# NJU-LHRS/LHRS-Bot

Measured on AMD Instinct MI355X. Metric: stage-1 pretrain samples/sec (224^2 image + 128-tok caption), higher is better.
Workload: dtype bf16

## Files before the change

### include/lhrs_hip.h

```cpp
#ifndef LHRS_HIP_H
#define LHRS_HIP_H
#include <stdint.h>
#ifdef __cplusplus
extern "C" {
#endif

typedef uint16_t lhrs_bf16_t;

const char* lhrs_last_error(void);
int lhrs_abi_version(void);
const char* lhrs_target_arch(void);

int lhrs_gemm_bf16_nt(const void* A, int lda, const void* B, int ldb, void* C, int ldc, int M, int N, int K,
                      const void* bias, const void* residual, int ldr, int act, int out_f32, int accumulate,
                      float alpha, void* stream);

int lhrs_gemm_bf16_nt_lora(const void* A, int lda, const void* B, int ldb, const void* A2, int lda2, const void* B2, int ldb2,
                           int K2, void* C, int ldc, int M, int N, int K, const void* bias, const void* residual, int ldr,
                           int out_f32, int accumulate, float alpha, void* stream);
int lhrs_gemm_fp8_nt(const void* A8, long lda, const float* sa, const void* B8, long ldb, const float* sb, void* C, int ldc,
                     int M, int N, int K, const void* residual, int ldr, float alpha, void* stream);
int lhrs_gemm_fp8_nt_lora(const void* A8, long lda, const float* sa, const void* B8, long ldb, const float* sb, const void* A2,
                          int lda2, const void* B2, int ldb2, int K2, void* C, int ldc, int M, int N, int K,
                          const void* residual, int ldr, float alpha, void* stream);
// ... 72 lines not shown
int lhrs_layernorm_fwd(const void* x, long ldx, const void* gamma, const void* beta, void* y, long ldy, float* mean,
                       float* rstd, int rows, int cols, float eps, void* stream);
int lhrs_layernorm_bwd_nblk(int rows);
int lhrs_layernorm_bwd(const void* dy, long ld_dy, const void* x, long ldx, const void* gamma, const float* mean,
                       const float* rstd, const void* add, void* dx, long ld_dx, float* dgamma, float* dbeta,
                       float* partial, int accumulate, int rows, int cols, void* stream);
int lhrs_rmsnorm_fwd(const void* x, long ldx, const void* w, void* y, long ldy, float* rstd, int rows, int cols,
                     float eps, void* stream);
int lhrs_rmsnorm_bwd(const void* dy, const void* x, const void* w, const float* rstd, const void* add, void* dx,
                     int rows, int cols, float eps, void* stream);

int lhrs_seq_transpose(const void* in, long ld_in, void* out, int cols, int LT, const int* desc, int nseq, int use_kv,
                       void* stream);
int lhrs_attn_fwd(const void* q, long ldq, const void* k, long ldk, const void* v, long ldv, void* o, long ldo, float* lse,
                  const int* desc, int nseq, int H, int D, int max_q, int max_kv, int LTq, int causal, float scale,
                  void* stream);
int lhrs_attn_fwd_kmask(const void* q, long ldq, const void* k, long ldk, const void* v, long ldv, void* o, long ldo,
                        float* lse, const int* desc, int nseq, int H, int D, int max_q, int max_kv, int LTq,
                        int causal, float scale, const unsigned char* key_mask, long ld_mask, void* stream);
int lhrs_attn_delta(const void* o, long ldo, const void* dout, long ld_do, float* delta, const int* desc, int nseq, int H,
                    int D, int max_q, int LTq, void* stream);
int lhrs_attn_bwd(const void* q, long ldq, const void* k, long ldk, const void* v, long ldv, const void* dout,
                  long ld_do, const float* lse, const float* delta, void* dq, long ld_dq, void* dk, long ld_dk, void* dv,
                  long ld_dv, const int* desc, int nseq, int H, int D, int max_q, int max_kv, int LTq, int causal,
                  float scale, void* stream);
int lhrs_attn_bwd_rope(const void* q, long ldq, const void* k, long ldk, const void* v, long ldv, const void* dout,
                       long ld_do, const float* lse, const float* delta, void* dq, long ld_dq, void* dk, long ld_dk, void* dv,
                       long ld_dv, const int* desc, int nseq, int H, int D, int max_q, int max_kv, int LTq, int causal,
                       float scale, const float* cos_t, const float* sin_t, int pos_mod, int pos0, long rows, void* stream);
int lhrs_attn_bwd_o(const void* q, long ldq, const void* k, long ldk, const void* v, long ldv, const void* dout, long ld_do,
                    const void* o, long ldo, const float* lse, float* delta, void* dq, long ld_dq, void* dk, long ld_dk, void* dv,
                    long ld_dv, const int* desc, int nseq, int H, int D, int max_q, int max_kv, int LTq, int causal, float scale,
                    const float* cos_t, const float* sin_t, int pos_mod, int pos0, long rows, void* stream);

int lhrs_patchify(const float* rgb, void* out, int B, int img, int P, int KP, void* stream);
int lhrs_vit_assemble(const void* patch, const void* cls, const void* pos, void* out, int B, int NP, int dim,
                      void* stream);
int lhrs_rope(void* x, long ld, int rows, int nheads, int D, const float* cos_t, const float* sin_t, const int* pos_ids,
              int pos_mod, int pos0, int inverse, void* stream);
int lhrs_swiglu_fwd(const void* gate_up, void* act, long rows, int F, void* stream);
int lhrs_swiglu_bwd(const void* dact, const void* gate_up, void* dgate_up, long rows, int F, void* stream);
int lhrs_map(int op, const void* a, const void* b, void* out, long n, void* stream);
int lhrs_colsum_nsplit(int rows);
int lhrs_colsum(const void* x, long ld, float* out, float* partial, int rows, int cols, int accumulate, void* stream);
int lhrs_cast_f32_to_bf16(const float* in, void* out, long n, void* stream);
int lhrs_cast_bf16_to_f32(const void* in, float* out, long n, void* stream);
int lhrs_transpose(const void* in, long ld_in, void* out, long ld_out, int rows, int cols, int rows_pad, void* stream);
int lhrs_transpose_batched(const long* desc, int n, int total_tiles, void* stream);

int lhrs_pooler_build(const void* query, const void* img, void* t, void* kv, int B, int nq0, int nq1, int nq2, int ni0,
                      int ni1, int ni2, int dim, void* stream);
int lhrs_pooler_query_grad(const void* dt0, const void* dkv, float* dquery, int B, int nq0, int nq1, int nq2, int ni0,
                           int ni1, int ni2, int dim, int accumulate, void* stream);
int lhrs_copy_2d(void* dst, long dst_pitch_bytes, const void* src, long src_pitch_bytes, long width_bytes, long height,
                 void* stream);
int lhrs_debug_poison_lds(unsigned pattern, void* stream);

int lhrs_splice_fwd(const long* ids, const long* labels, const uint8_t* mask, const void* image, const void* embed,
                    void* out_embeds, long* out_labels, uint8_t* out_mask, int* img_pos, int B, int T, int NI, int dim,
                    int S, int vocab, void* stream);
int lhrs_splice_bwd(const void* d_embeds, const int* img_pos, void* d_image, int B, int NI, int dim, int S, void* stream);
int lhrs_splice_map_fwd(const long* ids, const int* src_tok, const int* src_img, const void* image, const void* embed, void* out_embeds, int B,
                        int T, int dim, int S, int vocab, void* stream);
int lhrs_splice_map_bwd(const void* d_embeds, const int* inv, void* d_image, int n_rows, int dim, void* stream);
int lhrs_gather_rows(const void* src, long ld_src, const int* idx, void* dst, long ld_dst, int n, int dim, void* stream);
int lhrs_scatter_rows(const void* src, long ld_src, const int* idx, void* dst, long ld_dst, int n, int dim, void* stream);
// ... 72 lines not shown
```

### lhrs_bot_amd/csrc/attention.hip

```cpp
#include "common.h"
#include <type_traits>

namespace {

struct AttnArgs {
  const bf16_t* q; const bf16_t* k; const bf16_t* v; const bf16_t* dout;
  long ldq, ldk, ldv, ldo, ld_do, ld_dq, ld_dk, ld_dv;
  bf16_t* o; bf16_t* dq; bf16_t* dk; bf16_t* dv;
  int LTq;
  float* lse;
  const float* delta;
  const int* desc;
  int H;
  float scale;
  const unsigned char* kmask;
  long ld_kmask;
  const float* rope_cos;
  const float* rope_sin;
  int rope_mod, rope_pos0;
  const bf16_t* o_in;
  long ld_oin;
  float* delta_w;
  int wide;
};

constexpr float NEG_INF = -__builtin_huge_valf();

template <int D>
__device__ __forceinline__ int swz(int row) {
  return D == 128 ? (((row & 7) << 1) | ((row >> 3) & 1)) : (row & 7);
}
template <int D>
__device__ __forceinline__ int rm_off(int row, int c) { return row * (D * 2) + ((c ^ swz<D>(row)) << 4); }

template <int D> struct TileRegs { uint4 v[64 * (D / 8) / 256]; };

template <int D>
__device__ __forceinline__ void tile_load(TileRegs<D>& r, const bf16_t* base, long ld, int row0, int len, int tid) {
  constexpr int CH = D / 8, N = 64 * CH / 256;
#pragma unroll
  for (int i = 0; i < N; ++i) {
    const int idx = tid + i * 256;
    const int gr = min(row0 + idx / CH, len - 1);
    r.v[i] = *reinterpret_cast<const uint4*>(base + (long)gr * ld + (idx % CH) * 8);
  }
}
template <int D>
__device__ __forceinline__ void tile_store(char* lds, const TileRegs<D>& r, int tid) {
  constexpr int CH = D / 8, N = 64 * CH / 256;
#pragma unroll
  for (int i = 0; i < N; ++i) {
    const int idx = tid + i * 256;
    *reinterpret_cast<uint4*>(lds + rm_off<D>(idx / CH, idx % CH)) = r.v[i];
  }
}
template <int D>
// ... 388 lines not shown
    for (int db = 0; db < DB; ++db) dv[db] = MFMA(join(alo[db], ahi[db]), p1, dv[db]);
    tr_wait<DB>(blo, bhi);
#pragma unroll
    for (int db = 0; db < DB; ++db) dk[db] = MFMA(join(blo[db], bhi[db]), d1, dk[db]);
  }
  if (key < kv_rows) {
    bf16_t* pk = a.dk + (long)(kv_off + key) * a.ld_dk + h * D + fg * 4;
    bf16_t* pv = a.dv + (long)(kv_off + key) * a.ld_dv + h * D + fg * 4;
#pragma unroll
    for (int db = 0; db < DB; ++db) { store4bf(pk + db * 16, dk[db], 1.f); store4bf(pv + db * 16, dv[db], 1.f); }
  }
}

template <int D> constexpr int res_rows() { return 163840 / (2 * D * 2); }

template <int D>
__device__ __forceinline__ void res_load(char* lds, const bf16_t* base, long ld, int rows, int len, int lane, int wave) {
  constexpr int CH = D / 8, R = 1024 / (D * 2);
  typedef const __attribute__((address_space(1))) void* gp;
  typedef __attribute__((address_space(3))) void* lp;
  for (int r0 = wave * R; r0 < rows; r0 += 8 * R) {
    const int row = r0 + lane / CH;
    const int c = (lane % CH) ^ swz<D>(row);
    const bf16_t* src = base + (long)min(row, len - 1) * ld + c * 8;
    __builtin_amdgcn_global_load_lds((gp)src, (lp)(lds + r0 * (D * 2)), 16, 0, 0);
  }
}
__device__ __forceinline__ int zigzag_group(int p, int wave, int G, bool descending) {
  const int k = p * 8 + ((p & 1) ? 7 - wave : wave);
  if (k >= G) return -1;
  return descending ? G - 1 - k : k;
}

#ifdef ATTN_DIAG
__device__ unsigned long long* g_attn_dbg = nullptr;
__device__ int g_attn_dbg_sel = 0;
#define DIAG_T(slot) do { if (g_attn_dbg && g_attn_dbg_sel == DIAG_KID && lane == 0) g_attn_dbg[((long)(blockIdx.y * gridDim.x + blockIdx.x) * 8 + wave) * 8 + (slot)] = wall_clock64(); } while (0)
#define DIAG_DECL(id) constexpr int DIAG_KID = id; unsigned long long dg_t = 0, dg_acc[3] = {0, 0, 0}; int dg_units = 0
#define DIAG_MARK() do { asm volatile("s_waitcnt vmcnt(0) lgkmcnt(0)" ::: "memory"); dg_t = wall_clock64(); } while (0)
#define DIAG_ACC(k) do { asm volatile("s_waitcnt vmcnt(0) lgkmcnt(0)" ::: "memory"); const unsigned long long t_ = wall_clock64(); dg_acc[k] += t_ - dg_t; dg_t = t_; } while (0)
#define DIAG_UNITS(n) dg_units += (n)
#define DIAG_FLUSH() do { if (g_attn_dbg && g_attn_dbg_sel == DIAG_KID && lane == 0) { unsigned long long* d_ = g_attn_dbg + ((long)(blockIdx.y * gridDim.x + blockIdx.x) * 8 + wave) * 8; d_[2] = dg_acc[0]; d_[3] = dg_acc[1]; d_[5] = dg_acc[2]; d_[6] = dg_units; } } while (0)
#else
#define DIAG_T(slot) do { } while (0)
#define DIAG_DECL(id)
#define DIAG_MARK() do { } while (0)
#define DIAG_ACC(k) do { } while (0)
#define DIAG_UNITS(n) do { } while (0)
#define DIAG_FLUSH() do { } while (0)
#endif

template <int D, bool CAUSAL>
__global__ __launch_bounds__(512, 2) void attn_fwd_res_kernel(AttnArgs a) {
  constexpr int KS = D / 32, DB = D / 16, TILE = 64 * D * 2;
  __shared__ __attribute__((aligned(16))) char smem[163840];
  char* lds_k = smem;
  char* lds_v = smem + res_rows<D>() * D * 2;
  const int seq = blockIdx.y, h = blockIdx.x;
  const int* ds = a.desc + seq * 8;
  const int q_off = ds[0], q_len = ds[1], kv_off = ds[2], kv_len = ds[3], coff = ds[5];
  const int tid = threadIdx.x, lane = tid & 63, fr = lane & 15, fg = lane >> 4;
  const int wave = __builtin_amdgcn_readfirstlane(tid >> 6);
  DIAG_DECL(0);
  DIAG_T(0);
  int kv_need = kv_len;
  if (CAUSAL) kv_need = max(0, min(kv_len, q_len + coff));
  const int rows = ((kv_need + 63) >> 6) << 6;
  if (rows > 0) {
    res_load<D>(lds_k, a.k + (long)kv_off * a.ldk + h * D, a.ldk, rows, kv_len, lane, wave);
    res_load<D>(lds_v, a.v + (long)kv_off * a.ldv + h * D, a.ldv, rows, kv_len, lane, wave);
  }
  asm volatile("s_waitcnt vmcnt(0)" ::: "memory");
  __syncthreads();
  DIAG_T(1);
  TrAddr<D> tv;
  tv.init(lds_v, lane);
  const float c2 = a.scale * 1.4426950408889634f;
  const int G = (q_len + 15) >> 4;
  for (int p = 0;; ++p) {
    const int g = zigzag_group(p, wave, G, CAUSAL);
    if (g < 0) break;
    DIAG_MARK();
    const int qrow = g * 16 + fr;
    const bf16_t* qp = a.q + (long)(q_off + min(qrow, q_len - 1)) * a.ldq + h * D;
    bf16x8 qf[KS];
#pragma unroll
    for (int ks = 0; ks < KS; ++ks) qf[ks] = *reinterpret_cast<const bf16x8*>(qp + ks * 32 + fg * 8);
    DIAG_ACC(0);
    float m = NEG_INF, l = 0.f;
    f32x4 o[DB];
#pragma unroll
    for (int i = 0; i < DB; ++i) o[i] = f32x4{0.f, 0.f, 0.f, 0.f};
    int kv_end = kv_len;
    if (CAUSAL) kv_end = max(0, min(kv_len, min(g * 16 + 16, q_len) + coff));
    const int ntiles = (kv_end + 63) >> 6;
    for (int j = 0; j < ntiles; ++j) {
      const char* kt = lds_k + j * TILE;
      f32x4 s[4];
#pragma unroll
      for (int nb = 0; nb < 4; ++nb) {
        s[nb] = f32x4{0.f, 0.f, 0.f, 0.f};
#pragma unroll
        for (int ks = 0; ks < KS; ++ks) s[nb] = MFMA(frag_rm<D>(kt, nb * 16 + fr, ks, fg), qf[ks], s[nb]);
      }
      TrAddr<D> tj;
#pragma unroll
      for (int db = 0; db < DB; ++db) tj.base[db] = tv.base[db] + j * TILE;
      bf16x4 v0lo[DB], v0hi[DB], v1lo[DB], v1hi[DB];
      tr_issue<D, 0>(tj, v0lo, v0hi);
      const bool full = (j + 1) * 64 <= kv_len && (!CAUSAL || j * 64 + 63 <= g * 16 + coff);
// ... 24 lines not shown
        for (int r = 0; r < 4; ++r) {
          s[nb][r] = __builtin_amdgcn_exp2f(__builtin_fmaf(s[nb][r], c2, -mc));
          rs += s[nb][r];
        }
      l = l * alpha + rs;
      m = m_new;
#pragma unroll
      for (int i = 0; i < DB; ++i) o[i] *= alpha;
      const bf16x8 p0 = pack_frag(s[0], s[1]), p1 = pack_frag(s[2], s[3]);
      tr_wait<DB>(v0lo, v0hi);
      tr_issue<D, 1>(tj, v1lo, v1hi);
      __builtin_amdgcn_sched_barrier(0);
#pragma unroll
      for (int db = 0; db < DB; ++db) o[db] = MFMA(join(v0lo[db], v0hi[db]), p0, o[db]);
      tr_wait<DB>(v1lo, v1hi);
#pragma unroll
      for (int db = 0; db < DB; ++db) o[db] = MFMA(join(v1lo[db], v1hi[db]), p1, o[db]);
    }
    DIAG_ACC(1);
    DIAG_UNITS(ntiles);
    l = group_sum(l);
    if (qrow < q_len) {
      const float inv = l > 0.f ? 1.f / l : 0.f;
      bf16_t* op = a.o + (long)(q_off + qrow) * a.ldo + h * D;
      if (a.wide) store_row_wide<DB>(op, o, inv, fg);
      else {
#pragma unroll
        for (int db = 0; db < DB; ++db) store4bf(op + fg * 4 + db * 16, o[db], inv);
      }
      if (a.lse && fg == 0) a.lse[(long)(seq * a.H + h) * a.LTq + qrow] = (l > 0.f) ? m * a.scale + __logf(l) : NEG_INF;
    }
    DIAG_ACC(2);
  }
  DIAG_T(4);
  DIAG_FLUSH();
}

template <int D, bool CAUSAL>
__global__ __launch_bounds__(512, 2) void attn_bwd_dq_res_kernel(AttnArgs a) {
  constexpr int KS = D / 32, DB = D / 16, TILE = 64 * D * 2;
  __shared__ __attribute__((aligned(16))) char smem[163840];
  char* lds_k = smem;
  char* lds_v = smem + res_rows<D>() * D * 2;
  const int seq = blockIdx.y, h = blockIdx.x;
  const int* ds = a.desc + seq * 8;
  const int q_off = ds[0], q_len = ds[1], kv_off = ds[2], kv_len = ds[3], coff = ds[5];
  const int tid = threadIdx.x, lane = tid & 63, fr = lane & 15, fg = lane >> 4;
  const int wave = __builtin_amdgcn_readfirstlane(tid >> 6);
  DIAG_DECL(1);
  DIAG_T(0);
  int kv_need = kv_len;
  if (CAUSAL) kv_need = max(0, min(kv_len, q_len + coff));
  const int rows = ((kv_need + 63) >> 6) << 6;
  if (rows > 0) {
    res_load<D>(lds_k, a.k + (long)kv_off * a.ldk + h * D, a.ldk, rows, kv_len, lane, wave);
    res_load<D>(lds_v, a.v + (long)kv_off * a.ldv + h * D, a.ldv, rows, kv_len, lane, wave);
  }
  asm volatile("s_waitcnt vmcnt(0)" ::: "memory");
  __syncthreads();
  DIAG_T(1);
  TrAddr<D> tk;
  tk.init(lds_k, lane);
  const int G = (q_len + 15) >> 4;
  for (int p = 0;; ++p) {
    const int g = zigzag_group(p, wave, G, CAUSAL);
    if (g < 0) break;
    DIAG_MARK();
    const int qrow = g * 16 + fr;
    const int qrow_c = min(qrow, q_len - 1);
    const bf16_t* qp = a.q + (long)(q_off + qrow_c) * a.ldq + h * D;
    const bf16_t* dop = a.dout + (long)(q_off + qrow_c) * a.ld_do + h * D;
    bf16x8 qf[KS], dof[KS];
#pragma unroll
    for (int ks = 0; ks < KS; ++ks) {
      qf[ks] = *reinterpret_cast<const bf16x8*>(qp + ks * 32 + fg * 8);
      dof[ks] = *reinterpret_cast<const bf16x8*>(dop + ks * 32 + fg * 8);
    }
    const long stat = (long)(seq * a.H + h) * a.LTq + qrow_c;
    float delta_q;
    if (a.o_in != nullptr) {
      const bf16_t* op = a.o_in + (long)(q_off + qrow_c) * a.ld_oin + h * D;
      float part = 0.f;
#pragma unroll
      for (int ks = 0; ks < KS; ++ks) {
        const bf16x8 of = *reinterpret_cast<const bf16x8*>(op + ks * 32 + fg * 8);
#pragma unroll
        for (int e = 0; e < 8; ++e) part += bf2f((bf16_t)dof[ks][e]) * bf2f((bf16_t)of[e]);
      }
      delta_q = group_sum(part);
      if (fg == 0 && qrow < q_len) a.delta_w[stat] = delta_q;
    } else {
      delta_q = a.delta[stat];
    }
    const float lse2 = a.lse[stat] * 1.4426950408889634f, c2 = a.scale * 1.4426950408889634f;
    DIAG_ACC(0);
    f32x4 dq[DB];
#pragma unroll
    for (int i = 0; i < DB; ++i) dq[i] = f32x4{0.f, 0.f, 0.f, 0.f};
    int kv_end = kv_len;
    if (CAUSAL) kv_end = max(0, min(kv_len, min(g * 16 + 16, q_len) + coff));
    const int ntiles = (kv_end + 63) >> 6;
    for (int j = 0; j < ntiles; ++j) {
      const char* kt = lds_k + j * TILE;
      const char* vt = lds_v + j * TILE;
      f32x4 s[4], dp[4];
#pragma unroll
      for (int nb = 0; nb < 4; ++nb) {
        s[nb] = f32x4{0.f, 0.f, 0.f, 0.f};
        dp[nb] = f32x4{0.f, 0.f, 0.f, 0.f};
#pragma unroll
        for (int ks = 0; ks < KS; ++ks) {
          s[nb] = MFMA(frag_rm<D>(kt, nb * 16 + fr, ks, fg), qf[ks], s[nb]);
          dp[nb] = MFMA(frag_rm<D>(vt, nb * 16 + fr, ks, fg), dof[ks], dp[nb]);
        }
      }
      TrAddr<D> tj;
#pragma unroll
      for (int db = 0; db < DB; ++db) tj.base[db] = tk.base[db] + j * TILE;
      bf16x4 k0lo[DB], k0hi[DB], k1lo[DB], k1hi[DB];
      tr_issue<D, 0>(tj, k0lo, k0hi);
      const bool full = (j + 1) * 64 <= kv_len && (!CAUSAL || j * 64 + 63 <= g * 16 + coff);
      if (full) {
#pragma unroll
        for (int nb = 0; nb < 4; ++nb)
#pragma unroll
          for (int r = 0; r < 4; ++r) {
            const float pv = __builtin_amdgcn_exp2f(__builtin_fmaf(s[nb][r], c2, -lse2));
// ... 5 lines not shown
#pragma unroll
          for (int r = 0; r < 4; ++r) {
            const int key = j * 64 + nb * 16 + fg * 4 + r;
            const bool ok = key < kv_len && (!CAUSAL || key <= qrow + coff) && qrow < q_len;
            const float pv = __builtin_amdgcn_exp2f(__builtin_fmaf(s[nb][r], c2, -lse2));
            s[nb][r] = ok ? pv * (dp[nb][r] - delta_q) : 0.f;
          }
      }
      const bf16x8 d0 = pack_frag(s[0], s[1]), d1 = pack_frag(s[2], s[3]);
      tr_wait<DB>(k0lo, k0hi);
      tr_issue<D, 1>(tj, k1lo, k1hi);
      __builtin_amdgcn_sched_barrier(0);
#pragma unroll
      for (int db = 0; db < DB; ++db) dq[db] = MFMA(join(k0lo[db], k0hi[db]), d0, dq[db]);
      tr_wait<DB>(k1lo, k1hi);
#pragma unroll
      for (int db = 0; db < DB; ++db) dq[db] = MFMA(join(k1lo[db], k1hi[db]), d1, dq[db]);
    }
    DIAG_ACC(1);
    DIAG_UNITS(ntiles);
    if (qrow < q_len) {
#pragma unroll
      for (int db = 0; db < DB; ++db) dq[db] *= a.scale;
      if (a.rope_cos != nullptr) rope_bwd_inplace<DB>(dq, a, (long)q_off + qrow, fg);
      bf16_t* pq = a.dq + (long)(q_off + qrow) * a.ld_dq + h * D;
      if (a.wide) store_row_wide<DB>(pq, dq, 1.f, fg);
      else {
#pragma unroll
        for (int db = 0; db < DB; ++db) store4bf(pq + fg * 4 + db * 16, dq[db], 1.f);
      }
    }
    DIAG_ACC(2);
  }
  DIAG_T(4);
  DIAG_FLUSH();
}

template <int D, bool CAUSAL>
__global__ __launch_bounds__(512, 2) void attn_bwd_dkv_res_kernel(AttnArgs a) {
  constexpr int KS = D / 32, DB = D / 16, TILE = 64 * D * 2;
  __shared__ __attribute__((aligned(16))) char smem[163840];
  char* lds_q = smem;
  char* lds_do = smem + res_rows<D>() * D * 2;
  const int seq = blockIdx.y, h = blockIdx.x;
  const int* ds = a.desc + seq * 8;
  const int q_off = ds[0], q_len = ds[1], kv_off = ds[2], kv_len = ds[3], kv_rows = ds[4], coff = ds[5];
  const int tid = threadIdx.x, lane = tid & 63, fr = lane & 15, fg = lane >> 4;
  const int wave = __builtin_amdgcn_readfirstlane(tid >> 6);
  DIAG_DECL(2);
  DIAG_T(0);
  const int nq_tiles = (q_len + 63) >> 6;
  const bool half_last = nq_tiles > 0 && q_len - (nq_tiles - 1) * 64 <= 32;
  const int rows_alloc = nq_tiles * 64 - (half_last ? 32 : 0);
  float* lds_lse = reinterpret_cast<float*>(smem + rows_alloc * D * 2);
  float* lds_delta = lds_lse + a.LTq;
  const float* lsebase = a.lse + (long)(seq * a.H + h) * a.LTq;
  const float* deltabase = a.delta + (long)(seq * a.H + h) * a.LTq;
  res_load<D>(lds_q, a.q + (long)q_off * a.ldq + h * D, a.ldq, rows_alloc, q_len, lane, wave);
  res_load<D>(lds_do, a.dout + (long)q_off * a.ld_do + h * D, a.ld_do, rows_alloc, q_len, lane, wave);
  for (int t = tid; t < a.LTq; t += 512) { lds_lse[t] = lsebase[t]; lds_delta[t] = deltabase[t]; }
  asm volatile("s_waitcnt vmcnt(0)" ::: "memory");
  __syncthreads();
  DIAG_T(1);
  TrAddr<D> tq, tdo;
  tq.init(lds_q, lane);
  tdo.init(lds_do, lane);
  const int G = (kv_rows + 15) >> 4;
  for (int p = 0;; ++p) {
    const int g = zigzag_group(p, wave, G, !CAUSAL);
    if (g < 0) break;
    DIAG_MARK();
    const int key = g * 16 + fr;
    const int key_c = min(key, kv_rows - 1);
    const bf16_t* kp = a.k + (long)(kv_off + key_c) * a.ldk + h * D;
    const bf16_t* vp = a.v + (long)(kv_off + key_c) * a.ldv + h * D;
    bf16x8 kf[KS], vf[KS];
#pragma unroll
    for (int ks = 0; ks < KS; ++ks) {
      kf[ks] = *reinterpret_cast<const bf16x8*>(kp + ks * 32 + fg * 8);
      vf[ks] = *reinterpret_cast<const bf16x8*>(vp + ks * 32 + fg * 8);
    }
    f32x4 dk[DB], dv[DB];
#pragma unroll
    for (int i = 0; i < DB; ++i) { dk[i] = f32x4{0.f, 0.f, 0.f, 0.f}; dv[i] = f32x4{0.f, 0.f, 0.f, 0.f}; }
    int i0 = 0;
    if (CAUSAL) i0 = max(0, (g * 16 - coff) >> 6);
    DIAG_ACC(0);
    DIAG_UNITS(nq_tiles - i0);
    for (int i = i0; i < nq_tiles; ++i) {
      const bool hf = half_last && i == nq_tiles - 1;
      const char* qt = lds_q + i * TILE;
      const char* dot = lds_do + i * TILE;
      f32x4 s[4], dp[4];
#pragma unroll
      for (int qb = 0; qb < 2; ++qb) {
        s[qb] = f32x4{0.f, 0.f, 0.f, 0.f};
        dp[qb] = f32x4{0.f, 0.f, 0.f, 0.f};
#pragma unroll
        for (int ks = 0; ks < KS; ++ks) {
// ... 51 lines not shown
#pragma unroll
      for (int db = 0; db < DB; ++db) dk[db] = MFMA(join(alo[db], ahi[db]), d0, dk[db]);
      __builtin_amdgcn_sched_barrier(0);
      if (!hf) {
        probs(2); probs(3);
        const bf16x8 p1 = pack_frag(s[2], s[3]), d1 = pack_frag(dp[2], dp[3]);
        tr_issue<D, 1>(tdi, alo, ahi);
        tr_wait<DB>(alo, ahi);
#pragma unroll
        for (int db = 0; db < DB; ++db) dv[db] = MFMA(join(alo[db], ahi[db]), p1, dv[db]);
        __builtin_amdgcn_sched_barrier(0);
        tr_issue<D, 1>(tqi, alo, ahi);
        tr_wait<DB>(alo, ahi);
#pragma unroll
        for (int db = 0; db < DB; ++db) dk[db] = MFMA(join(alo[db], ahi[db]), d1, dk[db]);
        __builtin_amdgcn_sched_barrier(0);
      }
    }
    RopeRow<DB> rr;
    const bool rope = a.rope_cos != nullptr;
    if (rope) rope_row_load<DB>(rr, a, (long)kv_off + key_c, fg);
    DIAG_ACC(1);
    if (key < kv_rows) {
      if (rope) rope_row_apply<DB>(dk, rr);
      bf16_t* pk = a.dk + (long)(kv_off + key) * a.ld_dk + h * D;
      bf16_t* pv = a.dv + (long)(kv_off + key) * a.ld_dv + h * D;
      if (a.wide) { store_row_wide<DB>(pk, dk, 1.f, fg); store_row_wide<DB>(pv, dv, 1.f, fg); }
      else {
#pragma unroll
        for (int db = 0; db < DB; ++db) { store4bf(pk + fg * 4 + db * 16, dk[db], 1.f); store4bf(pv + fg * 4 + db * 16, dv[db], 1.f); }
      }
    }
    DIAG_ACC(2);
  }
  DIAG_T(4);
  DIAG_FLUSH();
}

template <int D>
__global__ void attn_delta_kernel(const bf16_t* __restrict__ o, long ldo, const bf16_t* __restrict__ dout, long ld_do,
                                  float* __restrict__ delta, const int* __restrict__ desc, int H, int LTq) {
  constexpr int TPR = D / 8;
  const int seq = blockIdx.z, h = blockIdx.y;
  const int q_off = desc[seq * 8 + 0], q_len = desc[seq * 8 + 1];
  const int t = blockIdx.x * (256 / TPR) + threadIdx.x / TPR;
  const int c = threadIdx.x % TPR;
  float s = 0.f;
  if (t < q_len) {
    const uint4 a = *reinterpret_cast<const uint4*>(o + (long)(q_off + t) * ldo + h * D + c * 8);
    const uint4 b = *reinterpret_cast<const uint4*>(dout + (long)(q_off + t) * ld_do + h * D + c * 8);
    s = bflo(a.x) * bflo(b.x) + bfhi(a.x) * bfhi(b.x) + bflo(a.y) * bflo(b.y) + bfhi(a.y) * bfhi(b.y) +
        bflo(a.z) * bflo(b.z) + bfhi(a.z) * bfhi(b.z) + bflo(a.w) * bflo(b.w) + bfhi(a.w) * bfhi(b.w);
  }
#pragma unroll
  for (int off = TPR / 2; off > 0; off >>= 1) s += __shfl_xor(s, off, 64);
  if (t < q_len && c == 0) delta[(long)(seq * H + h) * LTq + t] = s;
}

__global__ __launch_bounds__(256) void seq_transpose_kernel(const bf16_t* __restrict__ in, long ld_in, bf16_t* __restrict__ out,
                                                            int cols, int LT, const int* __restrict__ desc, int off_idx,
                                                            int len_idx) {
  __shared__ bf16_t tile[64][66];
  const int seq = blockIdx.z;
  const int off = desc[seq * 8 + off_idx], len = desc[seq * 8 + len_idx];
  const int t0 = blockIdx.x * 64, c0 = blockIdx.y * 64;
  const int tx = threadIdx.x & 63, ty = threadIdx.x >> 6;
// ... 3 lines not shown
  }
  __syncthreads();
  for (int r = ty; r < 64; r += 4) {
    const int c = c0 + r, t = t0 + tx;
    if (c < cols && t < LT) out[((long)seq * cols + c) * LT + t] = tile[tx][r];
  }
}

int check_common(const AttnArgs& a, int D, int nseq, const char* who) {
  LHRS_REQUIRE(D == 64 || D == 128, "%s: head_dim %d unsupported (64 or 128)", who, D);
  LHRS_REQUIRE(nseq > 0 && a.H > 0, "%s: nseq=%d H=%d", who, nseq, a.H);
  LHRS_REQUIRE(a.LTq % 64 == 0, "%s: LTq must be a multiple of 64", who);
  return 0;
}

}

#ifdef ATTN_DIAG
extern "C" int lhrs_attn_set_dbg(void* p, int sel) {
  unsigned long long* v = (unsigned long long*)p;
  if (hipMemcpyToSymbol(HIP_SYMBOL(g_attn_dbg_sel), &sel, sizeof(sel)) != hipSuccess) return -1;
  return hipMemcpyToSymbol(HIP_SYMBOL(g_attn_dbg), &v, sizeof(v)) == hipSuccess ? 0 : -1;
}
#endif
extern "C" int lhrs_seq_transpose(const void* in, long ld_in, void* out, int cols, int LT, const int* desc, int nseq,
                                  int use_kv, void* stream) {
  LHRS_REQUIRE(LT % 64 == 0 && cols > 0 && nseq > 0, "seq_transpose: LT=%d cols=%d nseq=%d", LT, cols, nseq);
  hipLaunchKernelGGL(seq_transpose_kernel, dim3(LT / 64, cdiv(cols, 64), nseq), dim3(256), 0, (hipStream_t)stream,
                     (const bf16_t*)in, ld_in, (bf16_t*)out, cols, LT, desc, use_kv ? 2 : 0, use_kv ? (use_kv == 2 ? 4 : 3) : 1);
  LHRS_CHECK_LAUNCH("seq_transpose");
  return 0;
}

static int attn_fwd_impl(const void* q, long ldq, const void* k, long ldk, const void* v, long ldv, void* o, long ldo,
                         float* lse, const int* desc, int nseq, int H, int D, int max_q, int max_kv, int LTq,
                         int causal, float scale, const unsigned char* key_mask, long ld_mask, void* stream) {
  AttnArgs a; memset(&a, 0, sizeof(a));
  a.kmask = key_mask; a.ld_kmask = ld_mask;
  if (key_mask != nullptr) max_kv = 1 << 30;
  a.q = (const bf16_t*)q; a.ldq = ldq; a.k = (const bf16_t*)k; a.ldk = ldk; a.v = (const bf16_t*)v; a.ldv = ldv;
  a.o = (bf16_t*)o; a.ldo = ldo; a.lse = lse; a.desc = desc; a.H = H; a.LTq = LTq; a.scale = scale;
  a.wide = (ldo % 8 == 0 && (size_t)o % 16 == 0) ? 1 : 0;
  if (check_common(a, D, nseq, "attn_fwd")) return -1;
  const dim3 grid(cdiv(max_q, 64), H, nseq), blk(256);
  hipStream_t s = (hipStream_t)stream;
  if (max_kv > 0 && max_kv <= (D == 128 ? res_rows<128>() : res_rows<64>())) {
    const dim3 rg(H, nseq), rb(512);
    if (D == 128) {
      if (causal) hipLaunchKernelGGL((attn_fwd_res_kernel<128, true>), rg, rb, 0, s, a);
      else hipLaunchKernelGGL((attn_fwd_res_kernel<128, false>), rg, rb, 0, s, a);
    } else {
      if (causal) hipLaunchKernelGGL((attn_fwd_res_kernel<64, true>), rg, rb, 0, s, a);
      else hipLaunchKernelGGL((attn_fwd_res_kernel<64, false>), rg, rb, 0, s, a);
    }
    LHRS_CHECK_LAUNCH("attn_fwd_res");
    return 0;
  }
  if (D == 128) {
    if (causal) hipLaunchKernelGGL((attn_fwd_kernel<128, true>), grid, blk, 0, s, a);
    else hipLaunchKernelGGL((attn_fwd_kernel<128, false>), grid, blk, 0, s, a);
  } else {
    if (causal) hipLaunchKernelGGL((attn_fwd_kernel<64, true>), grid, blk, 0, s, a);
    else hipLaunchKernelGGL((attn_fwd_kernel<64, false>), grid, blk, 0, s, a);
  }
  LHRS_CHECK_LAUNCH("attn_fwd");
  return 0;
}

extern "C" int lhrs_attn_fwd(const void* q, long ldq, const void* k, long ldk, const void* v, long ldv, void* o, long ldo,
                             float* lse, const int* desc, int nseq, int H, int D, int max_q, int max_kv, int LTq,
                             int causal, float scale, void* stream) {
  return attn_fwd_impl(q, ldq, k, ldk, v, ldv, o, ldo, lse, desc, nseq, H, D, max_q, max_kv, LTq, causal, scale, nullptr, 0, stream);
}

extern "C" int lhrs_attn_fwd_kmask(const void* q, long ldq, const void* k, long ldk, const void* v, long ldv, void* o, long ldo,
                                   float* lse, const int* desc, int nseq, int H, int D, int max_q, int max_kv, int LTq,
                                   int causal, float scale, const unsigned char* key_mask, long ld_mask, void* stream) {
  LHRS_REQUIRE(key_mask != nullptr && ld_mask > 0, "attn_fwd_kmask: key_mask=%p ld_mask=%ld", (const void*)key_mask, ld_mask);
  return attn_fwd_impl(q, ldq, k, ldk, v, ldv, o, ldo, lse, desc, nseq, H, D, max_q, max_kv, LTq, causal, scale, key_mask, ld_mask, stream);
}
// ... 11 lines not shown
                       (const bf16_t*)dout, ld_do, delta, desc, H, LTq);
  LHRS_CHECK_LAUNCH("attn_delta");
  return 0;
}

extern "C" int lhrs_rope(void* x, long ld, int rows, int nheads, int D, const float* cos_t, const float* sin_t, const int* pos_ids, int pos_mod,
                         int pos0, int inverse, void* stream);

static int attn_bwd_impl(const void* q, long ldq, const void* k, long ldk, const void* v, long ldv,
                         const void* dout, long ld_do, const float* lse, const float* delta, void* dq, long ld_dq,
                         void* dk, long ld_dk, void* dv, long ld_dv, const int* desc, int nseq, int H, int D,
                         int max_q, int max_kv, int LTq, int causal, float scale, const float* rope_cos, const float* rope_sin,
                         int rope_mod, int rope_pos0, long rope_rows, void* stream, const void* o = nullptr, long ldo = 0) {
  AttnArgs a; memset(&a, 0, sizeof(a));
  if (o != nullptr) {
    const int rmax0 = D == 128 ? res_rows<128>() : res_rows<64>();
    if (max_kv <= rmax0) { a.o_in = (const bf16_t*)o; a.ld_oin = ldo; a.delta_w = const_cast<float*>(delta); }
    else if (lhrs_attn_delta(o, ldo, dout, ld_do, const_cast<float*>(delta), desc, nseq, H, D, max_q, LTq, stream)) return -1;
  }
  const bool rope = rope_cos != nullptr;
  const int rmax_ = D == 128 ? res_rows<128>() : res_rows<64>();
  const bool dkv_fits = max_q <= rmax_ && (long)((max_q + 31) / 32 * 32) * D * 2 + 2L * LTq * 4 <= (long)rmax_ * D * 2;
  const bool fuse_rope = rope && max_kv <= rmax_ && dkv_fits;
  if (fuse_rope) { a.rope_cos = rope_cos; a.rope_sin = rope_sin; a.rope_mod = rope_mod; a.rope_pos0 = rope_pos0; }
  a.q = (const bf16_t*)q; a.ldq = ldq; a.k = (const bf16_t*)k; a.ldk = ldk; a.v = (const bf16_t*)v; a.ldv = ldv;
  a.dout = (const bf16_t*)dout; a.ld_do = ld_do; a.lse = (float*)lse; a.delta = delta;
  a.dq = (bf16_t*)dq; a.ld_dq = ld_dq; a.dk = (bf16_t*)dk; a.ld_dk = ld_dk; a.dv = (bf16_t*)dv; a.ld_dv = ld_dv;
  a.desc = desc; a.H = H; a.LTq = LTq; a.scale = scale;
  a.wide = (ld_dq % 8 == 0 && ld_dk % 8 == 0 && ld_dv % 8 == 0 && ((size_t)dq | (size_t)dk | (size_t)dv) % 16 == 0) ? 1 : 0;
  if (check_common(a, D, nseq, "attn_bwd")) return -1;
  hipStream_t s = (hipStream_t)stream;
  const dim3 gq(cdiv(max_q, 64), H, nseq), gk(cdiv(max_kv, 64), H, nseq), blk(256);
  const int rmax = D == 128 ? res_rows<128>() : res_rows<64>();
  const dim3 rg(H, nseq), rb(512);
  bool dq_done = false, dkv_done = false;
  if (max_kv <= rmax) {
    if (D == 128) { if (causal) hipLaunchKernelGGL((attn_bwd_dq_res_kernel<128, true>), rg, rb, 0, s, a); else hipLaunchKernelGGL((attn_bwd_dq_res_kernel<128, false>), rg, rb, 0, s, a); }
    else { if (causal) hipLaunchKernelGGL((attn_bwd_dq_res_kernel<64, true>), rg, rb, 0, s, a); else hipLaunchKernelGGL((attn_bwd_dq_res_kernel<64, false>), rg, rb, 0, s, a); }
    dq_done = true;
  }
  if (dkv_fits) {
    if (D == 128) { if (causal) hipLaunchKernelGGL((attn_bwd_dkv_res_kernel<128, true>), rg, rb, 0, s, a); else hipLaunchKernelGGL((attn_bwd_dkv_res_kernel<128, false>), rg, rb, 0, s, a); }
    else { if (causal) hipLaunchKernelGGL((attn_bwd_dkv_res_kernel<64, true>), rg, rb, 0, s, a); else hipLaunchKernelGGL((attn_bwd_dkv_res_kernel<64, false>), rg, rb, 0, s, a); }
    dkv_done = true;
  }
  if (dq_done && dkv_done) { LHRS_CHECK_LAUNCH("attn_bwd_res"); return 0; }
#define LAUNCH_TILED(KERN, GRID)                                                                 \
  do {                                                                                           \
    if (D == 128) { if (causal) hipLaunchKernelGGL((KERN<128, true>), GRID, blk, 0, s, a); else hipLaunchKernelGGL((KERN<128, false>), GRID, blk, 0, s, a); } \
    else { if (causal) hipLaunchKernelGGL((KERN<64, true>), GRID, blk, 0, s, a); else hipLaunchKernelGGL((KERN<64, false>), GRID, blk, 0, s, a); }          \
  } while (0)
  if (!dq_done) LAUNCH_TILED(attn_bwd_dq_kernel, gq);
  if (!dkv_done) LAUNCH_TILED(attn_bwd_dkv_kernel, gk);
#undef LAUNCH_TILED
  LHRS_CHECK_LAUNCH("attn_bwd");
  if (rope) {
    if (lhrs_rope(dq, ld_dq, (int)rope_rows, H, D, rope_cos, rope_sin, nullptr, rope_mod, rope_pos0, 1, stream)) return -1;
    if (lhrs_rope(dk, ld_dk, (int)rope_rows, H, D, rope_cos, rope_sin, nullptr, rope_mod, rope_pos0, 1, stream)) return -1;
  }
  return 0;
}

extern "C" int lhrs_attn_bwd(const void* q, long ldq, const void* k, long ldk, const void* v, long ldv,
                             const void* dout, long ld_do, const float* lse, const float* delta, void* dq, long ld_dq,
                             void* dk, long ld_dk, void* dv, long ld_dv, const int* desc, int nseq, int H, int D,
                             int max_q, int max_kv, int LTq, int causal, float scale, void* stream) {
  return attn_bwd_impl(q, ldq, k, ldk, v, ldv, dout, ld_do, lse, delta, dq, ld_dq, dk, ld_dk, dv, ld_dv, desc, nseq, H, D, max_q, max_kv, LTq,
                       causal, scale, nullptr, nullptr, 1, 0, 0, stream);
}

extern "C" int lhrs_attn_bwd_rope(const void* q, long ldq, const void* k, long ldk, const void* v, long ldv,
                                  const void* dout, long ld_do, const float* lse, const float* delta, void* dq, long ld_dq,
                                  void* dk, long ld_dk, void* dv, long ld_dv, const int* desc, int nseq, int H, int D,
                                  int max_q, int max_kv, int LTq, int causal, float scale, const float* cos_t, const float* sin_t,
// ... 16 lines not shown
```

Before: 171.8.

## Make resident attention kernels persistent with next-pair K/V prefetch and launch stagger

Converts the LDS-resident attention forward, dq and dkv kernels from a (head, seq) grid into a 1-D persistent grid capped at the CU count. Each block loops over (seq, head) pairs. For D=64 dq, the next pair's K/V is prefetched into registers during the current pair's compute. Blocks also get a start stagger based on s_sleep phases to spread out memory bursts. A per-kernel/per-head-dim table picks which kernels run persistent, and a runtime toggle is exposed. The intent is to cut tail and launch waves and overlap global loads with compute, at the cost of extra register pressure, sleep delay and serialized pairs per CU.

```diff
diff --git a/include/lhrs_hip.h b/include/lhrs_hip.h
--- a/include/lhrs_hip.h
+++ b/include/lhrs_hip.h
@@ -128,6 +128,7 @@
                     const void* o, long ldo, const float* lse, float* delta, void* dq, long ld_dq, void* dk, long ld_dk, void* dv,
                     long ld_dv, const int* desc, int nseq, int H, int D, int max_q, int max_kv, int LTq, int causal, float scale,
                     const float* cos_t, const float* sin_t, int pos_mod, int pos0, long rows, void* stream);
+int lhrs_attn_set_persistent(int on);
 
 int lhrs_patchify(const float* rgb, void* out, int B, int img, int P, int KP, void* stream);
 int lhrs_vit_assemble(const void* patch, const void* cls, const void* pos, void* out, int B, int NP, int dim,
diff --git a/lhrs_bot_amd/csrc/attention.hip b/lhrs_bot_amd/csrc/attention.hip
--- a/lhrs_bot_amd/csrc/attention.hip
+++ b/lhrs_bot_amd/csrc/attention.hip
@@ -1,5 +1,6 @@
 #include "common.h"
 #include <type_traits>
+#include <utility>
 
 namespace {
 
@@ -22,6 +23,7 @@
   long ld_oin;
   float* delta_w;
   int wide;
+  int npairs;
 };
 
 constexpr float NEG_INF = -__builtin_huge_valf();
@@ -476,6 +478,64 @@
   return descending ? G - 1 - k : k;
 }
 
+typedef unsigned int u32x4 __attribute__((ext_vector_type(4)));
+template <int D> struct ResStage {
+  static constexpr int N = res_rows<D>() / (8 * (1024 / (D * 2)));
+  u32x4 v[N];
+};
+template <int D, int I>
+__device__ __forceinline__ void stage_load1(ResStage<D>& s, const bf16_t* base, long ld, int rows, int len, int lane, int wave) {
+  constexpr int CH = D / 8, R = 1024 / (D * 2);
+  const int r0 = wave * R + I * 8 * R;
+  if (r0 < rows) {
+    const int row = r0 + lane / CH;
+    const int c = (lane % CH) ^ swz<D>(row);
+    s.v[I] = *reinterpret_cast<const u32x4*>(base + (long)min(row, len - 1) * ld + c * 8);
+  }
+}
+template <int D, int I>
+__device__ __forceinline__ void stage_store1(char* lds, const ResStage<D>& s, int rows, int lane, int wave) {
+  constexpr int R = 1024 / (D * 2);
+  const int r0 = wave * R + I * 8 * R;
+  if (r0 < rows) *reinterpret_cast<u32x4*>(lds + r0 * (D * 2) + lane * 16) = s.v[I];
+}
+template <int D, int... I>
+__device__ __forceinline__ void stage_load_seq(ResStage<D>& s, const bf16_t* base, long ld, int rows, int len, int lane, int wave, std::integer_sequence<int, I...>) {
+  (stage_load1<D, I>(s, base, ld, rows, len, lane, wave), ...);
+}
+template <int D, int... I>
+__device__ __forceinline__ void stage_store_seq(char* lds, const ResStage<D>& s, int rows, int lane, int wave, std::integer_sequence<int, I...>) {
+  (stage_store1<D, I>(lds, s, rows, lane, wave), ...);
+}
+template <int D>
+__device__ __forceinline__ void stage_load(ResStage<D>& s, const bf16_t* base, long ld, int rows, int len, int lane, int wave) {
+  stage_load_seq<D>(s, base, ld, rows, len, lane, wave, std::make_integer_sequence<int, ResStage<D>::N>{});
+}
+template <int D>
+__device__ __forceinline__ void stage_store(char* lds, const ResStage<D>& s, int rows, int lane, int wave) {
+  stage_store_seq<D>(lds, s, rows, lane, wave, std::make_integer_sequence<int, ResStage<D>::N>{});
+}
+__device__ __forceinline__ int stage_lane(int lane) {
+  asm volatile("" : "+v"(lane));
+  return lane;
+}
+template <int KS>
+__device__ __forceinline__ void frag_arrived(bf16x8 (&f)[KS]) {
+  if constexpr (KS == 4) asm volatile("" : "+v"(f[0]), "+v"(f[1]), "+v"(f[2]), "+v"(f[3]) : : "memory");
+  else {
+    static_assert(KS == 2, "frag_arrived: head_dim 64 or 128");
+    asm volatile("" : "+v"(f[0]), "+v"(f[1]) : : "memory");
+  }
+  __builtin_amdgcn_sched_barrier(0);
+}
+
+constexpr int STAGGER_PHASES = 4;
+__device__ __forceinline__ void stagger(int npairs, int period_us) {
+  if ((int)gridDim.x < npairs) {
+    const int n = (int)((blockIdx.x >> 3) & (STAGGER_PHASES - 1)) * period_us * 4 / STAGGER_PHASES;
+    for (int i = 0; i < n; ++i) __builtin_amdgcn_s_sleep(8);
+  }
+}
 #ifdef ATTN_DIAG
 __device__ unsigned long long* g_attn_dbg = nullptr;
 __device__ int g_attn_dbg_sel = 0;
@@ -500,13 +560,15 @@
   __shared__ __attribute__((aligned(16))) char smem[163840];
   char* lds_k = smem;
   char* lds_v = smem + res_rows<D>() * D * 2;
-  const int seq = blockIdx.y, h = blockIdx.x;
+  int pr = blockIdx.x;
+  int seq = pr / a.H, h = pr - seq * a.H;
   const int* ds = a.desc + seq * 8;
-  const int q_off = ds[0], q_len = ds[1], kv_off = ds[2], kv_len = ds[3], coff = ds[5];
+  int q_off = ds[0], q_len = ds[1], kv_off = ds[2], kv_len = ds[3], coff = ds[5];
   const int tid = threadIdx.x, lane = tid & 63, fr = lane & 15, fg = lane >> 4;
   const int wave = __builtin_amdgcn_readfirstlane(tid >> 6);
   DIAG_DECL(0);
   DIAG_T(0);
+  stagger(a.npairs, 17);
   int kv_need = kv_len;
   if (CAUSAL) kv_need = max(0, min(kv_len, q_len + coff));
   const int rows = ((kv_need + 63) >> 6) << 6;
@@ -520,6 +582,18 @@
   TrAddr<D> tv;
   tv.init(lds_v, lane);
   const float c2 = a.scale * 1.4426950408889634f;
+  for (;;) {
+  const int nxt = pr + (int)gridDim.x;
+  const bool more = nxt < a.npairs;
+  int n_seq = 0, n_h = 0, n_q_off = 0, n_q_len = 0, n_kv_off = 0, n_kv_len = 0, n_coff = 0, n_rows = 0;
+  if (more) {
+    n_seq = nxt / a.H; n_h = nxt - n_seq * a.H;
+    const int* nd = a.desc + n_seq * 8;
+    n_q_off = nd[0]; n_q_len = nd[1]; n_kv_off = nd[2]; n_kv_len = nd[3]; n_coff = nd[5];
+    int n_need = n_kv_len;
+    if (CAUSAL) n_need = max(0, min(n_kv_len, n_q_len + n_coff));
+    n_rows = ((n_need + 63) >> 6) << 6;
+  }
   const int G = (q_len + 15) >> 4;
   for (int p = 0;; ++p) {
     const int g = zigzag_group(p, wave, G, CAUSAL);
@@ -610,6 +684,16 @@
     }
     DIAG_ACC(2);
   }
+  if (!more) break;
+  __syncthreads();
+  if (n_rows > 0) {
+    res_load<D>(lds_k, a.k + (long)n_kv_off * a.ldk + n_h * D, a.ldk, n_rows, n_kv_len, lane, wave);
+    res_load<D>(lds_v, a.v + (long)n_kv_off * a.ldv + n_h * D, a.ldv, n_rows, n_kv_len, lane, wave);
+  }
+  asm volatile("s_waitcnt vmcnt(0)" ::: "memory");
+  __syncthreads();
+  pr = nxt; seq = n_seq; h = n_h; q_off = n_q_off; q_len = n_q_len; kv_off = n_kv_off; kv_len = n_kv_len; coff = n_coff;
+  }
   DIAG_T(4);
   DIAG_FLUSH();
 }
@@ -620,13 +704,16 @@
   __shared__ __attribute__((aligned(16))) char smem[163840];
   char* lds_k = smem;
   char* lds_v = smem + res_rows<D>() * D * 2;
-  const int seq = blockIdx.y, h = blockIdx.x;
+  constexpr bool STAGE = D == 64;
+  int pr = blockIdx.x;
+  int seq = pr / a.H, h = pr - seq * a.H;
   const int* ds = a.desc + seq * 8;
-  const int q_off = ds[0], q_len = ds[1], kv_off = ds[2], kv_len = ds[3], coff = ds[5];
+  int q_off = ds[0], q_len = ds[1], kv_off = ds[2], kv_len = ds[3], coff = ds[5];
   const int tid = threadIdx.x, lane = tid & 63, fr = lane & 15, fg = lane >> 4;
   const int wave = __builtin_amdgcn_readfirstlane(tid >> 6);
   DIAG_DECL(1);
   DIAG_T(0);
+  if (!STAGE) stagger(a.npairs, 27);
   int kv_need = kv_len;
   if (CAUSAL) kv_need = max(0, min(kv_len, q_len + coff));
   const int rows = ((kv_need + 63) >> 6) << 6;
@@ -639,6 +726,27 @@
   DIAG_T(1);
   TrAddr<D> tk;
   tk.init(lds_k, lane);
+  for (;;) {
+  const int nxt = pr + (int)gridDim.x;
+  const bool more = nxt < a.npairs;
+  int n_seq = 0, n_h = 0, n_q_off = 0, n_q_len = 0, n_kv_off = 0, n_kv_len = 0, n_coff = 0, n_rows = 0;
+  if (more) {
+    n_seq = nxt / a.H; n_h = nxt - n_seq * a.H;
+    const int* nd = a.desc + n_seq * 8;
+    n_q_off = nd[0]; n_q_len = nd[1]; n_kv_off = nd[2]; n_kv_len = nd[3]; n_coff = nd[5];
+    int n_need = n_kv_len;
+    if (CAUSAL) n_need = max(0, min(n_kv_len, n_q_len + n_coff));
+    n_rows = ((n_need + 63) >> 6) << 6;
+  }
+  ResStage<D> sk, sv;
+  bool staged = !more || !STAGE;
+  auto stage = [&]() __attribute__((always_inline)) {
+    const int ln = stage_lane(lane);
+    stage_load<D>(sk, a.k + (long)n_kv_off * a.ldk + n_h * D, a.ldk, n_rows, n_kv_len, ln, wave);
+    stage_load<D>(sv, a.v + (long)n_kv_off * a.ldv + n_h * D, a.ldv, n_rows, n_kv_len, ln, wave);
+    __builtin_amdgcn_sched_barrier(0);
+    staged = true;
+  };
   const int G = (q_len + 15) >> 4;
   for (int p = 0;; ++p) {
     const int g = zigzag_group(p, wave, G, CAUSAL);
@@ -670,7 +778,14 @@
     } else {
       delta_q = a.delta[stat];
     }
-    const float lse2 = a.lse[stat] * 1.4426950408889634f, c2 = a.scale * 1.4426950408889634f;
+    float lse2 = a.lse[stat] * 1.4426950408889634f;
+    const float c2 = a.scale * 1.4426950408889634f;
+    if (!staged) {
+      asm volatile("" : "+v"(lse2), "+v"(delta_q) : : "memory");
+      frag_arrived<KS>(qf);
+      frag_arrived<KS>(dof);
+      stage();
+    }
     DIAG_ACC(0);
     f32x4 dq[DB];
 #pragma unroll
@@ -742,6 +857,22 @@
     }
     DIAG_ACC(2);
   }
+  if (!more) break;
+  if (!staged) stage();
+  __syncthreads();
+  if constexpr (STAGE) {
+    stage_store<D>(lds_k, sk, n_rows, lane, wave);
+    stage_store<D>(lds_v, sv, n_rows, lane, wave);
+  } else {
+    if (n_rows > 0) {
+      res_load<D>(lds_k, a.k + (long)n_kv_off * a.ldk + n_h * D, a.ldk, n_rows, n_kv_len, lane, wave);
+      res_load<D>(lds_v, a.v + (long)n_kv_off * a.ldv + n_h * D, a.ldv, n_rows, n_kv_len, lane, wave);
+    }
+    asm volatile("s_waitcnt vmcnt(0)" ::: "memory");
+  }
+  __syncthreads();
+  pr = nxt; seq = n_seq; h = n_h; q_off = n_q_off; q_len = n_q_len; kv_off = n_kv_off; kv_len = n_kv_len; coff = n_coff;
+  }
   DIAG_T(4);
   DIAG_FLUSH();
 }
@@ -752,11 +883,18 @@
   __shared__ __attribute__((aligned(16))) char smem[163840];
   char* lds_q = smem;
   char* lds_do = smem + res_rows<D>() * D * 2;
-  const int seq = blockIdx.y, h = blockIdx.x;
+  int pr = blockIdx.x;
+  int seq = pr / a.H, h = pr - seq * a.H;
   const int* ds = a.desc + seq * 8;
-  const int q_off = ds[0], q_len = ds[1], kv_off = ds[2], kv_len = ds[3], kv_rows = ds[4], coff = ds[5];
-  const int tid = threadIdx.x, lane = tid & 63, fr = lane & 15, fg = lane >> 4;
+  int q_off = ds[0], q_len = ds[1], kv_off = ds[2], kv_len = ds[3], kv_rows = ds[4], coff = ds[5];
+  const int tid = threadIdx.x;
   const int wave = __builtin_amdgcn_readfirstlane(tid >> 6);
+  TrAddr<D> tq, tdo;
+  tq.init(lds_q, tid & 63);
+  tdo.init(lds_do, tid & 63);
+  stagger(a.npairs, 31);
+  for (;;) {
+  const int lane = stage_lane(tid & 63), fr = lane & 15, fg = lane >> 4;
   DIAG_DECL(2);
   DIAG_T(0);
   const int nq_tiles = (q_len + 63) >> 6;
@@ -766,15 +904,23 @@
   float* lds_delta = lds_lse + a.LTq;
   const float* lsebase = a.lse + (long)(seq * a.H + h) * a.LTq;
   const float* deltabase = a.delta + (long)(seq * a.H + h) * a.LTq;
-  res_load<D>(lds_q, a.q + (long)q_off * a.ldq + h * D, a.ldq, rows_alloc, q_len, lane, wave);
-  res_load<D>(lds_do, a.dout + (long)q_off * a.ld_do + h * D, a.ld_do, rows_alloc, q_len, lane, wave);
-  for (int t = tid; t < a.LTq; t += 512) { lds_lse[t] = lsebase[t]; lds_delta[t] = deltabase[t]; }
-  asm volatile("s_waitcnt vmcnt(0)" ::: "memory");
-  __syncthreads();
+  {
+    const int t0 = stage_lane(tid);
+    res_load<D>(lds_q, a.q + (long)q_off * a.ldq + h * D, a.ldq, rows_alloc, q_len, lane, wave);
+    res_load<D>(lds_do, a.dout + (long)q_off * a.ld_do + h * D, a.ld_do, rows_alloc, q_len, lane, wave);
+    for (int t = t0; t < a.LTq; t += 512) { lds_lse[t] = lsebase[t]; lds_delta[t] = deltabase[t]; }
+    asm volatile("s_waitcnt vmcnt(0)" ::: "memory");
+    __syncthreads();
+  }
   DIAG_T(1);
-  TrAddr<D> tq, tdo;
-  tq.init(lds_q, lane);
-  tdo.init(lds_do, lane);
+  const int nxt = pr + (int)gridDim.x;
+  const bool more = nxt < a.npairs;
+  int n_seq = 0, n_h = 0;
+  if (more) {
+    n_seq = nxt / a.H; n_h = nxt - n_seq * a.H;
+    const int warm = a.desc[n_seq * 8];
+    asm volatile("" : : "s"(warm));
+  }
   const int G = (kv_rows + 15) >> 4;
   for (int p = 0;; ++p) {
     const int g = zigzag_group(p, wave, G, !CAUSAL);
@@ -892,6 +1038,12 @@
       }
     }
     DIAG_ACC(2);
+  }
+  if (!more) break;
+  __syncthreads();
+  pr = nxt; seq = n_seq; h = n_h;
+  const int* nd = a.desc + seq * 8;
+  q_off = nd[0]; q_len = nd[1]; kv_off = nd[2]; kv_len = nd[3]; kv_rows = nd[4]; coff = nd[5];
   }
   DIAG_T(4);
   DIAG_FLUSH();
@@ -961,6 +1113,20 @@
   return 0;
 }
 
+static int g_attn_persist = 1;
+extern "C" int lhrs_attn_set_persistent(int on) { g_attn_persist = on; return 0; }
+enum { RES_FWD = 0, RES_DQ = 1, RES_DKV = 2 };
+static dim3 res_grid(int kernel, int D, int npairs) {
+  static int cus = 0;
+  if (cus == 0) {
+    int dev = 0;
+    if (hipGetDevice(&dev) != hipSuccess || hipDeviceGetAttribute(&cus, hipDeviceAttributeMultiprocessorCount, dev) != hipSuccess || cus <= 0) cus = 256;
+  }
+  static const bool keep[3][2] = {{false, true}, {true, false}, {false, true}};
+  const bool on = g_attn_persist == 2 || (g_attn_persist != 0 && keep[kernel][D == 128]);
+  return dim3((unsigned)(on && npairs > cus ? cus : npairs));
+}
+
 static int attn_fwd_impl(const void* q, long ldq, const void* k, long ldk, const void* v, long ldv, void* o, long ldo,
                          float* lse, const int* desc, int nseq, int H, int D, int max_q, int max_kv, int LTq,
                          int causal, float scale, const unsigned char* key_mask, long ld_mask, void* stream) {
@@ -974,7 +1140,8 @@
   const dim3 grid(cdiv(max_q, 64), H, nseq), blk(256);
   hipStream_t s = (hipStream_t)stream;
   if (max_kv > 0 && max_kv <= (D == 128 ? res_rows<128>() : res_rows<64>())) {
-    const dim3 rg(H, nseq), rb(512);
+    const dim3 rg = res_grid(RES_FWD, D, H * nseq), rb(512);
+    a.npairs = H * nseq;
     if (D == 128) {
       if (causal) hipLaunchKernelGGL((attn_fwd_res_kernel<128, true>), rg, rb, 0, s, a);
       else hipLaunchKernelGGL((attn_fwd_res_kernel<128, false>), rg, rb, 0, s, a);
@@ -1052,14 +1219,17 @@
   hipStream_t s = (hipStream_t)stream;
   const dim3 gq(cdiv(max_q, 64), H, nseq), gk(cdiv(max_kv, 64), H, nseq), blk(256);
   const int rmax = D == 128 ? res_rows<128>() : res_rows<64>();
-  const dim3 rg(H, nseq), rb(512);
+  const dim3 rb(512);
+  a.npairs = H * nseq;
   bool dq_done = false, dkv_done = false;
   if (max_kv <= rmax) {
+    const dim3 rg = res_grid(RES_DQ, D, H * nseq);
     if (D == 128) { if (causal) hipLaunchKernelGGL((attn_bwd_dq_res_kernel<128, true>), rg, rb, 0, s, a); else hipLaunchKernelGGL((attn_bwd_dq_res_kernel<128, false>), rg, rb, 0, s, a); }
     else { if (causal) hipLaunchKernelGGL((attn_bwd_dq_res_kernel<64, true>), rg, rb, 0, s, a); else hipLaunchKernelGGL((attn_bwd_dq_res_kernel<64, false>), rg, rb, 0, s, a); }
     dq_done = true;
   }
   if (dkv_fits) {
+    const dim3 rg = res_grid(RES_DKV, D, H * nseq);
     if (D == 128) { if (causal) hipLaunchKernelGGL((attn_bwd_dkv_res_kernel<128, true>), rg, rb, 0, s, a); else hipLaunchKernelGGL((attn_bwd_dkv_res_kernel<128, false>), rg, rb, 0, s, a); }
     else { if (causal) hipLaunchKernelGGL((attn_bwd_dkv_res_kernel<64, true>), rg, rb, 0, s, a); else hipLaunchKernelGGL((attn_bwd_dkv_res_kernel<64, false>), rg, rb, 0, s, a); }
     dkv_done = true;
```

Result: no change. 172.0, median of 3 (+0.1%).
